# NeurAI-Lab/biHomE

Hardware: AMD Instinct MI355X
Metric: training image-pairs/s (128x128 patch, bs=64 per GPU, full step: fwd+bwd+Adam) (higher is better)
Workload: dtype f32

## Files before the change

bihome_amd/_lib.py:

```python
import ctypes
import os
from ctypes import POINTER, Structure, c_char_p, c_float, c_int, c_int64, c_void_p

_HERE = os.path.dirname(os.path.abspath(__file__))
TUNING = os.environ.get("BIHOME_TUNING") == "1"
_VARIANT = os.environ.get("BIHOME_LIB_VARIANT", "")
LIB_PATH = os.path.join(_HERE, "libbihome_hip_tuning.so" if TUNING else
                        ("libbihome_hip_%s.so" % _VARIANT if _VARIANT.isalnum() else "libbihome_hip.so"))


class BhConvDesc(Structure):
    _fields_ = [(n, c_int) for n in ("N", "Hi", "Wi", "Ci", "Ho", "Wo", "Co", "kh", "kw", "stride", "pad",
                                     "transposed", "in_nchw", "out_nchw", "precision", "w_layout", "route")] + \
               [("a_bound", c_void_p), ("b_bound", c_void_p)]


GEOMETRY_FIELDS = tuple(n for n, _ in BhConvDesc._fields_[:17])
AMAX_FLOATS = 512


class BhPack3x3Job(Structure):
    _fields_ = [("w", c_void_p), ("pf", c_void_p), ("pd", c_void_p), ("Co", c_int), ("Ci", c_int), ("split", c_int),
                ("reserved", c_int)]

# ... 44 lines not shown
    "bh_l2norm_bwd": [P, P, P, c_int, c_int, P, P],
    "bh_relu_bwd": [P, P, c_int64, P, P],
    "bh_oneline_anchor_bwd": [P] * 8 + [c_int, c_int, c_int, c_int, P, c_int, P, P, P],
    "bh_bihome_anchor_bwd": [P] * 10 + [c_int, c_int, c_int, c_float, c_int, P, P, P],
    "bh_warp_bwd_img": [P, P, c_int, c_int, c_int, c_int, P, P, c_int, P],
    "bh_photo_warp_fwd": [P, P, P, c_int, c_int, c_int, c_int, c_int, P, c_int, P],
    "bh_photo_warp_bwd": [P, P, P, P, c_int, c_int, c_int, c_int, c_int, P, c_int, P],
    "bh_mask_fwd": [P, P, c_int, c_int, c_float, P, P, P, P, P],
    "bh_mask_bwd": [P] * 7 + [c_int, c_int, c_float, P, P, P],
    "bh_conv3x3_pack": [P, c_int, P],
    "bh_conv3x3_pack_f16": [P, c_int, P],
    "bh_absmax": [P, c_int64, P, P],
    "bh_bn_fwd_coeffs": [P, P, P, P, P, c_int, c_int, c_int, c_float, c_float, P, P, P],
    "bh_bn_fwd": [P] * 8 + [c_int, c_int, c_int, c_float, c_float, c_int, c_int, P, P],
    "bh_bn_bwd": [P] * 11 + [c_int, c_int, c_int, c_float, c_int, c_int, P, P, P, P],
    "bh_conv_variant": [POINTER(BhConvDesc), c_int, c_int, c_int, c_char_p, c_int],
    "bh_conv_fwd": [P, P, P, P, POINTER(BhConvDesc), P],
    "bh_conv_fwd_act": [P, P, P, P, P, POINTER(BhConvDesc), c_int, P],
    "bh_conv_fwd_amax": [P, P, P, P, POINTER(BhConvDesc), P, P],
    "bh_conv_fwd_bnstats": [P, P, P, P, POINTER(BhConvDesc), P, c_int, P],
    "bh_conv_fwd_bnin": [P, P, P, P, POINTER(BhConvDesc), P, c_int, POINTER(BhBnIn), P],
    "bh_conv_wgrad_bnin": [P, P, P, P, POINTER(BhConvDesc), P, c_int64, POINTER(BhBnIn), P],
    "bh_conv_dgrad": [P, P, P, POINTER(BhConvDesc), c_int, P],
    "bh_conv_dgrad_colsum": [P, P, P, POINTER(BhConvDesc), P, P],
    "bh_bias_grad_from_sums": [P, P, c_int, c_int, P],
    "bh_conv_dgrad_s2": [P, P, P, POINTER(BhConvDesc), c_int, P, P],
    "bh_conv_dgrad_bnreduce": [P, P, P, POINTER(BhConvDesc), c_int, POINTER(BhBnReduce), P, c_int, P],
    "bh_col2im_c1": [P, P, POINTER(BhConvDesc), c_int, P],
    "bh_stem7_dgrad_c1": [P, P, P, POINTER(BhConvDesc), P],
    "bh_stem7_dgrad_c1_warp": [P, P, P, POINTER(BhConvDesc), P, P, P, c_int, P, P],
# ... 74 lines not shown
```

bihome_amd/csrc/bn.hip:

```cpp
#include "common.h"

#define BN_MAX_CHUNKS 256

struct BnGeom {
    int groups, rows, C, C4, LPR, RPP, nchunks, rows_per_chunk;
    int det;
};

static bool bn_geom(int groups, int rows, int C, BnGeom& g, int det) {
    if (C % 4 || groups < 1 || rows < 1) return false;
    g.groups = groups; g.rows = rows; g.C = C; g.C4 = C / 4; g.det = det;
    if (g.C4 > 256 || (256 % g.C4)) return false;
    g.LPR = g.C4; g.RPP = 256 / g.LPR;
    int n = rows / (g.RPP * 4);
    if (n < 1) n = 1;
    if (n > BN_MAX_CHUNKS) n = BN_MAX_CHUNKS;
    g.rows_per_chunk = (rows + n - 1) / n;
    g.nchunks = (rows + g.rows_per_chunk - 1) / g.rows_per_chunk;
    return true;
}

template <int NV>
__device__ __forceinline__ void reduce_rows(double (&v)[NV], int LPR, int RPP, double* sm ) {
    for (int i = 0; i < NV; ++i) sm[threadIdx.x * NV + i] = v[i];
// ... 82 lines not shown
}
__device__ __forceinline__ void bn_coeffs_from_raw(const BnRaw& r, int use_running, float eps, double inv_rows, float& mean,
                                                   float& invstd, float& scale, float& shift) {
    if (use_running) { mean = (float)r.s1; invstd = 1.0f / sqrtf((float)r.s2 + eps); }
    else {
        const double m = r.s1 * inv_rows;
        double var = r.s2 * inv_rows - m * m;
        if (var < 0) var = 0;
        mean = (float)m;
        invstd = 1.0f / sqrtf((float)var + eps);
    }
    scale = r.gm * invstd;
    shift = r.bt - mean * scale;
}

__global__ void __launch_bounds__(256) bn_apply_kernel(const float* __restrict__ x, const float* __restrict__ gamma,
                                                       const float* __restrict__ beta, const float* __restrict__ rmean,
                                                       const float* __restrict__ rvar, const float* __restrict__ res,
                                                       float* __restrict__ y, const double* __restrict__ stats, BnGeom g,
                                                       float eps, int flags, int use_running, float momentum,
                                                       float* __restrict__ upd_mean, float* __restrict__ upd_var,
                                                       unsigned* __restrict__ amax) {
    __shared__ float sm_amax[4];
    float vmax = 0.f;
    const int cq = threadIdx.x % g.LPR, r0 = threadIdx.x / g.LPR;
    const int grp = blockIdx.y;
    BnRaw raw[4];
#pragma unroll
    for (int i = 0; i < 4; ++i) raw[i] = bn_raw(stats, gamma, beta, rmean, rvar, use_running, g.groups, grp, g.C, cq * 4 + i, g.det);
    const size_t gbase = ((size_t)grp * g.rows) * g.C + cq * 4;
    const bool relu = flags & 1, addres = (flags & 2) && res;
    const int stride = gridDim.x * g.RPP;
    int r = blockIdx.x * g.RPP + r0;
    float4 a[4], q[4];
#pragma unroll
    for (int u = 0; u < 4; ++u) {
        const int rr = r + u * stride;
// ... 3 lines not shown
    float sc[4], sh[4];
    const double inv_rows = 1.0 / (double)g.rows;
#pragma unroll
    for (int i = 0; i < 4; ++i) {
        float m, is;
        bn_coeffs_from_raw(raw[i], use_running, eps, inv_rows, m, is, sc[i], sh[i]);
    }
    if (upd_mean && blockIdx.x == 0 && blockIdx.y == 0) bn_update_running(stats, g, momentum, upd_mean, upd_var);
    while (true) {
#pragma unroll
        for (int u = 0; u < 4; ++u) {
            const int rr = r + u * stride;
            if (rr >= g.rows) break;
            float4 o = make_float4(a[u].x * sc[0] + sh[0], a[u].y * sc[1] + sh[1], a[u].z * sc[2] + sh[2], a[u].w * sc[3] + sh[3]);
            if (addres) { o.x += q[u].x; o.y += q[u].y; o.z += q[u].z; o.w += q[u].w; }
            if (relu) { o.x = fmaxf(o.x, 0.f); o.y = fmaxf(o.y, 0.f); o.z = fmaxf(o.z, 0.f); o.w = fmaxf(o.w, 0.f); }
            *reinterpret_cast<float4*>(y + gbase + (size_t)rr * g.C) = o;
            vmax = fmaxf(fmaxf(vmax, fmaxf(fabsf(o.x), fabsf(o.y))), fmaxf(fabsf(o.z), fabsf(o.w)));
        }
        r += 4 * stride;
        if (r >= g.rows) break;
#pragma unroll
        for (int u = 0; u < 4; ++u) {
            const int rr = r + u * stride;
            a[u] = rr < g.rows ? *reinterpret_cast<const float4*>(x + gbase + (size_t)rr * g.C) : make_float4(0.f, 0.f, 0.f, 0.f);
            q[u] = (addres && rr < g.rows) ? *reinterpret_cast<const float4*>(res + gbase + (size_t)rr * g.C) : make_float4(0.f, 0.f, 0.f, 0.f);
        }
    }
    if (amax) bh_amax_commit(amax, vmax, blockIdx.x + blockIdx.y * 7u, sm_amax);
}

__global__ void __launch_bounds__(256) bn_bwd_reduce_kernel(const float* __restrict__ gy, const float* __restrict__ y,
                                                            const float* __restrict__ x, const float* __restrict__ gamma,
                                                            const float* __restrict__ beta, const double* __restrict__ stats,
                                                            const float* __restrict__ rmean, const float* __restrict__ rvar,
                                                            BnGeom g, float eps, int flags, int use_running,
                                                            double* __restrict__ part) {
    __shared__ double sm[256 * 8];
    const int cq = threadIdx.x % g.LPR, r0 = threadIdx.x / g.LPR;
    const int grp = blockIdx.y, chunk = blockIdx.x;
    const int rbeg = chunk * g.rows_per_chunk, rend = min(g.rows, rbeg + g.rows_per_chunk);
    float mean[4], invstd[4], sc[4], sh[4];
#pragma unroll
    for (int i = 0; i < 4; ++i)
        bn_coeffs(stats, gamma, beta, rmean, rvar, use_running, g.groups, grp, g.C, cq * 4 + i, eps, (double)g.rows, mean[i], invstd[i], sc[i], sh[i], g.det);
    const size_t gbase = ((size_t)grp * g.rows) * g.C + cq * 4;
    const bool relu = flags & 1, mask_from_x = flags & 4;
    double v[8] = {0, 0, 0, 0, 0, 0, 0, 0};
    const bool need_y = relu && !mask_from_x;
    auto accumulate = [&](float4 d, const float4& a, const float4& yv) {
        if (relu) {
            float4 o;
            if (mask_from_x) o = make_float4(a.x * sc[0] + sh[0], a.y * sc[1] + sh[1], a.z * sc[2] + sh[2], a.w * sc[3] + sh[3]);
            else o = yv;
            if (!(o.x > 0.f)) d.x = 0.f;
            if (!(o.y > 0.f)) d.y = 0.f;
            if (!(o.z > 0.f)) d.z = 0.f;
            if (!(o.w > 0.f)) d.w = 0.f;
        }
        v[0] += d.x; v[1] += d.y; v[2] += d.z; v[3] += d.w;
        v[4] += (double)(d.x * ((a.x - mean[0]) * invstd[0]));
        v[5] += (double)(d.y * ((a.y - mean[1]) * invstd[1]));
        v[6] += (double)(d.z * ((a.z - mean[2]) * invstd[2]));
        v[7] += (double)(d.w * ((a.w - mean[3]) * invstd[3]));
    };
    int r = rbeg + r0;
    for (; r + 3 * g.RPP < rend; r += 4 * g.RPP) {
        float4 d[4], a[4], yv[4];
#pragma unroll
        for (int u = 0; u < 4; ++u) {
            const size_t off = gbase + (size_t)(r + u * g.RPP) * g.C;
            d[u] = *reinterpret_cast<const float4*>(gy + off);
            a[u] = *reinterpret_cast<const float4*>(x + off);
            yv[u] = need_y ? *reinterpret_cast<const float4*>(y + off) : make_float4(0.f, 0.f, 0.f, 0.f);
        }
#pragma unroll
        for (int u = 0; u < 4; ++u) accumulate(d[u], a[u], yv[u]);
    }
    for (; r < rend; r += g.RPP) {
        const size_t off = gbase + (size_t)r * g.C;
        const float4 d = *reinterpret_cast<const float4*>(gy + off);
        const float4 a = *reinterpret_cast<const float4*>(x + off);
        const float4 yv = need_y ? *reinterpret_cast<const float4*>(y + off) : make_float4(0.f, 0.f, 0.f, 0.f);
        accumulate(d, a, yv);
    }
    reduce_rows<8>(v, g.LPR, g.RPP, sm);
    if ((int)threadIdx.x < g.LPR) {
        double* p = part + (((size_t)grp * g.nchunks + chunk) * g.C + cq * 4) * 2;
        for (int i = 0; i < 4; ++i) { p[i * 2] = v[i]; p[i * 2 + 1] = v[4 + i]; }
    }
}

__global__ void __launch_bounds__(64) bn_bwd_finalize_kernel(const double* __restrict__ part, BnGeom g,
                                                             const double* __restrict__ stats, const float* __restrict__ rmean,
                                                             const float* __restrict__ rvar, float eps, int use_running,
                                                             float* __restrict__ ggamma, float* __restrict__ gbeta,
                                                             float4* __restrict__ coef) {
    const int c = blockIdx.x, lane = threadIdx.x;
    double tg = 0, tb = 0;
// ... 7 lines not shown
        if (lane == 0) {
            float mean, invstd, sc, sh;
            bn_coeffs(stats, nullptr, nullptr, rmean, rvar, use_running, g.groups, grp, g.C, c, eps, (double)g.rows, mean, invstd, sc, sh, g.det);
            const float invn = 1.0f / (float)g.rows;
            coef[(size_t)grp * g.C + c] = use_running ? make_float4(mean, invstd, 0.f, 0.f)
                                                      : make_float4(mean, invstd, (float)s1 * invn, (float)s2 * invn);
        }
        tb += s1; tg += s2;
    }
    if (lane == 0) {
        if (ggamma) ggamma[c] += (float)tg;
        if (gbeta) gbeta[c] += (float)tb;
    }
}

__global__ void __launch_bounds__(256) bn_bwd_apply_kernel(const float* __restrict__ gy, const float* __restrict__ y,
                                                           const float* __restrict__ x, const float* __restrict__ gamma,
                                                           const float* __restrict__ beta,
                                                           const float4* __restrict__ coef,
                                                           float* __restrict__ gx, float* __restrict__ gres, BnGeom g,
                                                           int flags, const double* __restrict__ stats,
                                                           const double* __restrict__ sums, float eps,
                                                           float* __restrict__ ggamma, float* __restrict__ gbeta,
                                                           unsigned* __restrict__ amax) {
    __shared__ float sm_amax[4];
    float vmax = 0.f;
    const int cq = threadIdx.x % g.LPR, r0 = threadIdx.x / g.LPR;
    const int grp = blockIdx.y;
    BnRaw raw[4];
    float4 cf4[4];
    double rs1[4], rs2[4];
#pragma unroll
    for (int i = 0; i < 4; ++i) {
        const int c = cq * 4 + i;
        cf4[i] = make_float4(0.f, 0.f, 0.f, 0.f); rs1[i] = 0; rs2[i] = 0;
        if (coef) {
            cf4[i] = coef[(size_t)grp * g.C + c];
            raw[i].gm = gamma ? gamma[c] : 1.f; raw[i].bt = beta ? beta[c] : 0.f; raw[i].s1 = 0; raw[i].s2 = 0;
        } else {
            raw[i] = bn_raw(stats, gamma, beta, nullptr, nullptr, 0, g.groups, grp, g.C, c, g.det);
            rs1[i] = bn_sum_total(sums, g.groups, grp, g.C, c, 0, g.det);
            rs2[i] = bn_sum_total(sums, g.groups, grp, g.C, c, 1, g.det);
        }
    }
    const size_t gbase = ((size_t)grp * g.rows) * g.C + cq * 4;
    const bool relu = flags & 1, mask_from_x = flags & 4;
    const bool rd_y = relu && !mask_from_x;
    const int stride = gridDim.x * g.RPP;
    int r = blockIdx.x * g.RPP + r0;
    float4 dv[4], av[4], yv[4];
    auto issue = [&](int rb) {
#pragma unroll
        for (int u = 0; u < 4; ++u) {
            const int rr = rb + u * stride;
            const size_t off = gbase + (size_t)rr * g.C;
            const bool ok = rr < g.rows;
            dv[u] = ok ? *reinterpret_cast<const float4*>(gy + off) : make_float4(0.f, 0.f, 0.f, 0.f);
            av[u] = ok ? *reinterpret_cast<const float4*>(x + off) : make_float4(0.f, 0.f, 0.f, 0.f);
            yv[u] = (ok && rd_y) ? *reinterpret_cast<const float4*>(y + off) : make_float4(0.f, 0.f, 0.f, 0.f);
        }
    };
    issue(r);
    float mean[4], invstd[4], sc[4], sh[4], k1[4], k2[4];
    const double inv_rows = 1.0 / (double)g.rows;
    const float invn = 1.0f / (float)g.rows;
#pragma unroll
    for (int i = 0; i < 4; ++i) {
        if (coef) {
            mean[i] = cf4[i].x; invstd[i] = cf4[i].y; k1[i] = cf4[i].z; k2[i] = cf4[i].w;
            sc[i] = raw[i].gm * cf4[i].y;
            sh[i] = raw[i].bt - cf4[i].x * sc[i];
        } else {
            bn_coeffs_from_raw(raw[i], 0, eps, inv_rows, mean[i], invstd[i], sc[i], sh[i]);
            k1[i] = (float)rs1[i] * invn;
// ... 11 lines not shown
            if (gbeta) gbeta[c] += (float)tb;
        }
    }
    while (true) {
#pragma unroll
        for (int u = 0; u < 4; ++u) {
            const int rr = r + u * stride;
            if (rr >= g.rows) break;
            const size_t off = gbase + (size_t)rr * g.C;
            float4 d = dv[u];
            const float4 a = av[u];
            if (relu) {
                float4 o;
                if (mask_from_x) o = make_float4(a.x * sc[0] + sh[0], a.y * sc[1] + sh[1], a.z * sc[2] + sh[2], a.w * sc[3] + sh[3]);
                else o = yv[u];
                if (!(o.x > 0.f)) d.x = 0.f;
                if (!(o.y > 0.f)) d.y = 0.f;
                if (!(o.z > 0.f)) d.z = 0.f;
                if (!(o.w > 0.f)) d.w = 0.f;
            }
            if (gres) *reinterpret_cast<float4*>(gres + off) = d;
            float4 o;
            o.x = sc[0] * (d.x - k1[0] - (a.x - mean[0]) * invstd[0] * k2[0]);
            o.y = sc[1] * (d.y - k1[1] - (a.y - mean[1]) * invstd[1] * k2[1]);
            o.z = sc[2] * (d.z - k1[2] - (a.z - mean[2]) * invstd[2] * k2[2]);
            o.w = sc[3] * (d.w - k1[3] - (a.w - mean[3]) * invstd[3] * k2[3]);
            *reinterpret_cast<float4*>(gx + off) = o;
            vmax = fmaxf(fmaxf(vmax, fmaxf(fabsf(o.x), fabsf(o.y))), fmaxf(fabsf(o.z), fabsf(o.w)));
        }
        r += 4 * stride;
        if (r >= g.rows) break;
        issue(r);
    }
    if (amax) bh_amax_commit(amax, vmax, blockIdx.x + blockIdx.y * 7u, sm_amax);
// ... 338 lines not shown
}

int bn1_fwd(const float* x, const float* gamma, const float* beta, float* running_mean, float* running_var, const float* res, float* y,
            double* stats, int groups, int rows, float eps, float momentum, int flags, int use_running, hipStream_t s);
int bn1_bwd(const float* gy, const float* y, const float* x, const float* gamma, const float* beta, const double* stats, float* gx,
            float* gres, float* ggamma, float* gbeta, double* scratch, int groups, int rows, float eps, int flags, int use_running,
            const float* running_mean, const float* running_var, hipStream_t s);

extern "C" {

int bh_bn_stats_doubles(int groups, int C) { return (int)BH_BN_SUM_DOUBLES(groups, C); }

int bh_bn_fwd(const float* x, const float* gamma, const float* beta, float* running_mean, float* running_var,
              const float* res, float* y, double* stats, int groups, int rows, int C, float eps, float momentum,
              int flags, int use_running, float* amax_y, void* stream) {
    BnGeom g;
    if (!x || !y || !stats) return BH_E_BADARG;
    if (use_running && (!running_mean || !running_var)) return BH_E_BADARG;
    if (C == 1) return amax_y ? BH_E_UNSUPPORTED : bn1_fwd(x, gamma, beta, running_mean, running_var, res, y, stats, groups, rows, eps, momentum, flags, use_running, bh_stream(stream));
    if (!bn_geom(groups, rows, C, g, (flags & BH_BN_DETERMINISTIC) ? 1 : 0)) return BH_E_UNSUPPORTED;
    hipStream_t s = bh_stream(stream);
    if (!use_running && !(flags & 8)) {
        hipLaunchKernelGGL(bn_stats_kernel, dim3(g.nchunks, groups), dim3(256), 0, s, x, g, stats);
        BH_LAUNCH_CHECK();
    }
    const bool upd = !use_running && running_mean && running_var;
    hipLaunchKernelGGL(bn_apply_kernel, dim3(apply_blocks(g), groups), dim3(256), 0, s, x, gamma, beta, running_mean,
                       running_var, res, y, stats, g, eps, flags, use_running, momentum, upd ? running_mean : nullptr,
                       upd ? running_var : nullptr, reinterpret_cast<unsigned*>(amax_y));
    BH_LAUNCH_CHECK();
    return BH_OK;
}

int bh_bn_fwd_coeffs(const double* stats, const float* gamma, const float* beta, float* running_mean, float* running_var, int groups,
                     int rows, int C, float eps, float momentum, float* table, float* amax_y, void* stream) {
    BnGeom g;
    if (!stats || !table) return BH_E_BADARG;
    if (!bn_geom(groups, rows, C, g, -1)) return BH_E_UNSUPPORTED;
    const bool upd = running_mean && running_var;
    hipLaunchKernelGGL(bn_fwd_coeffs_kernel, dim3((groups * C + 255) / 256 + (upd ? 1 : 0)), dim3(256), 0, bh_stream(stream), stats, gamma, beta, g, eps,
                       momentum, upd ? running_mean : nullptr, upd ? running_var : nullptr, reinterpret_cast<float2*>(table),
                       reinterpret_cast<unsigned*>(amax_y));
    BH_LAUNCH_CHECK();
    return BH_OK;
}

int bh_bn_bwd(const float* gy, const float* y, const float* x, const float* gamma, const float* beta, const double* stats, float* gx,
              float* gres, float* ggamma, float* gbeta, double* scratch, int groups, int rows, int C, float eps, int flags,
              int use_running, const float* running_mean, const float* running_var, float* amax_gx, void* stream) {
    BnGeom g;
    if (!gy || !x || !gx || !stats || !scratch || ((flags & 1) && !(flags & 4) && !y)) return BH_E_BADARG;
    if ((flags & 4) && (flags & 2)) return BH_E_BADARG;
    if (C == 1) return amax_gx ? BH_E_UNSUPPORTED : bn1_bwd(gy, y, x, gamma, beta, stats, gx, gres, ggamma, gbeta, scratch, groups, rows, eps, flags, use_running,
                               running_mean, running_var, bh_stream(stream));
    if (!bn_geom(groups, rows, C, g, (flags & BH_BN_DETERMINISTIC) ? 1 : 0)) return BH_E_UNSUPPORTED;
    hipStream_t s = bh_stream(stream);
    if (flags & 16) {
        if (use_running) return BH_E_BADARG;
        hipLaunchKernelGGL(bn_bwd_apply_kernel, dim3(apply_blocks(g), groups), dim3(256), 0, s, gy, y, x, gamma, beta,
                           (const float4*)nullptr, gx, gres, g, flags, stats, (const double*)scratch, eps, ggamma, gbeta,
                           reinterpret_cast<unsigned*>(amax_gx));
        BH_LAUNCH_CHECK();
        return BH_OK;
    }
    float4* coef = reinterpret_cast<float4*>(scratch);
    double* part = scratch + (size_t)groups * C * 2;
    const bool need_sums = !use_running || ggamma || gbeta;
    if (need_sums) {
        hipLaunchKernelGGL(bn_bwd_reduce_kernel, dim3(g.nchunks, groups), dim3(256), 0, s, gy, y, x, gamma, beta, stats,
                           running_mean, running_var, g, eps, flags, use_running, part);
        BH_LAUNCH_CHECK();
    }
    BnGeom gf = g;
    if (!need_sums) gf.nchunks = 0;
    hipLaunchKernelGGL(bn_bwd_finalize_kernel, dim3(C), dim3(64), 0, s, part, gf, stats, running_mean, running_var, eps,
                       use_running, ggamma, gbeta, coef);
    BH_LAUNCH_CHECK();
    hipLaunchKernelGGL(bn_bwd_apply_kernel, dim3(apply_blocks(g), groups), dim3(256), 0, s, gy, y, x, gamma, beta, coef,
                       gx, gres, g, flags, (const double*)nullptr, (const double*)nullptr, eps, (float*)nullptr,
                       (float*)nullptr, reinterpret_cast<unsigned*>(amax_gx));
    BH_LAUNCH_CHECK();
    return BH_OK;
}

int bh_bn_scratch_doubles(int groups, int C) { return groups * C * 2 * (1 + (BN_MAX_CHUNKS > 256 ? BN_MAX_CHUNKS : 256)); }

int bh_bn_stats(const float* x, double* stats, int groups, int rows, int C, int flags, void* stream) {
    if (!x || !stats) return BH_E_BADARG;
    return bn_launch_stats(x, groups, rows, C, stats, bh_stream(stream), (flags & BH_BN_DETERMINISTIC) ? 1 : 0);
}

int bh_bn_maxpool_fwd(const float* x, const float* gamma, const float* beta, float* running_mean, float* running_var, float* y,
                      unsigned char* idx, double* stats, int groups, int N, int Hi, int Wi, int C, float eps, float momentum, int flags,
                      int use_running, float* amax_y, void* stream) {
    BnGeom g;
// ... 409 lines not shown
```

bihome_amd/kernels.py:

```python
import ctypes
import os

import torch

from ._lib import (AMAX_FLOATS, BN_DETERMINISTIC, DSAC_METHODS, F_DETERMINISTIC, GEOMETRY_FIELDS, ROUTE_DETERMINISTIC, ROUTE_WX3_PC, ROUTE_WX3_SHARED, BhBnIn, BhBnReduce, BhConvDesc,
                   BhPack3x3Job, check, lib)


def _p(t):
    return None if t is None else ctypes.c_void_p(t.data_ptr())


_DET_DEFAULT = os.environ.get("BIHOME_DETERMINISTIC", "0") == "1"
_DET_SCOPE = []


def set_deterministic(on=True):
    global _DET_DEFAULT
    prev, _DET_DEFAULT = _DET_DEFAULT, bool(on)
    return prev


def deterministic():
    return _DET_SCOPE[-1] if _DET_SCOPE else _DET_DEFAULT
# ... 984 lines not shown
            check(lib.bh_conv_bias_grad(_p(gy), _p(gbias), ctypes.byref(d), _stream()), "bh_conv_bias_grad")


BN_SUM_STRIDE = 16
BN_SUM_SLOTS = 1


def bn_stats_doubles(groups, C):
    return BN_SUM_SLOTS * groups * C * 2 * BN_SUM_STRIDE


def bn_stats_buffer(groups, C, device):
    return torch.zeros(lib.bh_bn_stats_doubles(groups, C), dtype=torch.float64, device=device)


def bn_fwd(x, gamma, beta, rmean, rvar, res, groups, eps, momentum, relu, training, stats=None, stats_ready=False, amax=None):
    _chk(x); _chk(res)
    C = gamma.numel() if gamma is not None else x.shape[-1]
    rows = x.numel() // C // groups
    y = torch.empty_like(x)
    if stats is None:
        stats = bn_stats_buffer(groups, C, x.device)
        stats_ready = False
    flags = (1 if relu else 0) | (2 if res is not None else 0) | (8 if stats_ready else 0) | (BN_DETERMINISTIC if deterministic() else 0)
    nb = 4.0 * x.numel() * ((2 if (training and not stats_ready) else 1) + 1 + (1 if res is not None else 0))
    with _Timed("bn_fwd(%d kernels)" % (2 if (training and not stats_ready) else 1) + (" g%d rows%d C%d" % (groups, rows, C) if TIMING_DETAIL else ""), 0.0, nb):
        check(lib.bh_bn_fwd(_p(x), _p(gamma), _p(beta), _p(rmean), _p(rvar), _p(res), _p(y), _p(stats), groups, rows, C,
                            float(eps), float(momentum), flags, 0 if training else 1, _p(amax), _stream()), "bh_bn_fwd")
    if amax is not None:
        y._bh_amax = amax
    return y, stats


def bn_bwd(gy, y, x, gamma, stats, rmean, rvar, groups, eps, relu, training, want_gres, ggamma=None, gbeta=None, beta=None,
           had_res=None, scratch=None, sums_ready=None, amax=None):
    _chk(gy); _chk(x)
    C = gamma.numel() if gamma is not None else x.shape[-1]
    rows = x.numel() // C // groups
    gx = torch.empty_like(x)
    gres = torch.empty_like(x) if want_gres else None
    if sums_ready is not None:
        scratch = sums_ready
    elif scratch is None:
        scratch = torch.empty(lib.bh_bn_scratch_doubles(groups, C), dtype=torch.float64, device=x.device)
    had_res = want_gres if had_res is None else had_res
    mask_from_x = relu and not had_res
    flags = ((1 if relu else 0) | (2 if want_gres else 0) | (4 if mask_from_x else 0) | (16 if sums_ready is not None else 0)
             | (BN_DETERMINISTIC if deterministic() else 0))
    passes = 1 if sums_ready is not None else 2
    nb = 4.0 * x.numel() * (passes * (2 + (1 if (relu and not mask_from_x) else 0)) + 1 + (1 if want_gres else 0))
    with _Timed("bn_bwd(%d kernels)" % (1 if sums_ready is not None else 3) + (" g%d rows%d C%d" % (groups, rows, C) if TIMING_DETAIL else ""), 0.0, nb):
        check(lib.bh_bn_bwd(_p(gy), _p(y), _p(x), _p(gamma), _p(beta), _p(stats), _p(gx), _p(gres), _p(ggamma), _p(gbeta),
                            _p(scratch), groups, rows, C, float(eps), flags, 0 if training else 1, _p(rmean), _p(rvar),
                            _p(amax), _stream()), "bh_bn_bwd")
    if amax is not None:
        gx._bh_amax = amax
    return gx, gres


def bn_stats(x, stats, groups, C):
    _chk(x); _chk(stats, torch.float64)
    rows = x.numel() // C // groups
    with _Timed("bn_stats_kernel", 0.0, 4.0 * x.numel()):
        check(lib.bh_bn_stats(_p(x), _p(stats), groups, rows, C, BN_DETERMINISTIC if deterministic() else 0, _stream()), "bh_bn_stats")
    return stats


class BnPooled:
    __slots__ = ("pooled", "idx", "shape")
# ... 200 lines not shown
```

bihome_amd/net.py:

```python
import os
import weakref

import torch
import torch.nn as nn

from . import kernels as K
from . import plan as P


def to_kernel_layout_(module):
    for m in module.modules():
        if isinstance(m, (nn.Conv2d, nn.ConvTranspose2d)):
            if not m.weight.data.is_contiguous(memory_format=torch.channels_last):
                m.weight.data = m.weight.data.contiguous(memory_format=torch.channels_last)
    return module


def kview(w):
    if w.dim() == 2:
        return w
    v = w.permute(0, 2, 3, 1)
    if not v.is_contiguous():
        raise RuntimeError("conv weight is not in kernel (channels_last) layout; call net.to_kernel_layout_(module)")
    return v
# ... 151 lines not shown
            low = self.sequential(src, blk.lower_branch)
        up = list(blk.upper_branch)
        assert isinstance(up[-1], nn.BatchNorm2d)
        mid = self.sequential(src, up[:-1])
        return self.bn(mid, up[-1], relu=True, res=low)

    def basic_block(self, src, blk):
        low = src
        if blk.downsample is not None:
            low = self.sequential(src, blk.downsample)
        t = self.bn(self.conv(src, blk.conv1), blk.bn1, relu=True)
        return self.bn(self.conv(t, blk.conv2), blk.bn2, relu=True, res=low)


class Ctx:
    __slots__ = ("slots", "stats", "descs", "groups", "training", "weights", "wkeys", "wpacked", "precision", "joined")

    def __init__(self):
        self.slots, self.stats, self.descs, self.weights, self.wkeys, self.wpacked = {}, {}, {}, {}, {}, {}
        self.joined = {}
        self.precision = 0


_GEOM_CACHE = {}
X3_WS_BYTES = 40 << 20
DET_WS_BYTES = 256 << 20


def _conv_geometry(mod, x_shape, in_nchw, out_nchw, precision=0):
    key = (id(mod), tuple(x_shape), bool(in_nchw), bool(out_nchw), int(precision), K.deterministic())
    hit = _GEOM_CACHE.get(key)
    if hit is not None and hit[0] is mod:
        return hit[1]
    d = _conv_geometry_uncached(mod, x_shape, in_nchw, out_nchw, precision)
    d.bh_packs = bool(isinstance(mod, nn.Conv2d) and K.packs_3x3(d))
# ... 153 lines not shown
    else:
        if isinstance(res, K.BnJoinPending):
            lo, _ = K.bn_fwd(res.x, res.mod.weight, res.mod.bias, res.mod.running_mean, res.mod.running_var, None, groups, res.mod.eps,
                             _momentum(res.mod), False, training, stats=res.stats, stats_ready=True)
            res = s.slots[op.res] = lo
        st = _bn_stats_slice(s, i, m.num_features)
        if i in plan.bn_pool and src.dim() == 4 and src.shape[0] % groups == 0:
            out = K.bn_maxpool_fwd(src, m.weight, m.bias, m.running_mean, m.running_var, groups, m.eps, _momentum(m), op.relu,
                                   training, st, i in s.ready, want_index=s.save, amax=amax_next() if amax_next else None)
        elif _bn_on_load_ok(s, i, op, src):
            rec = amax_next() if amax_next else None
            table = K.bn_fwd_coeffs(st, m.weight, m.bias, m.running_mean, m.running_var, groups,
                                    src.numel() // (m.num_features * groups), m.num_features, m.eps, _momentum(m), amax=rec)
            out = K.BnOnLoad(src, table, groups, op.relu, amax=rec)
        else:
            out, st = K.bn_fwd(src, m.weight, m.bias, m.running_mean, m.running_var, res, groups, m.eps, _momentum(m), op.relu, training,
                               stats=st, stats_ready=i in s.ready, amax=amax_next() if (amax_next and m.num_features > 1) else None)
    if training:
        _count_batch(m, groups)
    if s.save:
        s.ctx.stats[i] = st
    return out


def _fw_tail(s, i, op, src):
    c1, bn, c2 = op.mod
    N, h, w, _ = src.shape
    out, ws = K.tail_fwd(src, kview(c1.weight), c1.bias, bn.weight, bn.bias, bn.running_mean, bn.running_var,
                         kview(c2.weight), c2.bias, s.groups, h * w, bn.eps, _momentum(bn), s.training)
    if s.training:
        _count_batch(bn, s.groups)
    if s.save:
# ... 163 lines not shown
    train_w = s.want_wgrad and m.weight is not None and m.weight.requires_grad
    ggamma, gbeta = (m.weight.grad, m.bias.grad) if train_w else (None, None)
    amax = amax_next() if (amax_next and m.num_features > 1) else None
    gres = None
    if isinstance(g, K.GradFrom1x1):
        gx = K.bn_bwd_from_1x1(g, x, m.weight, m.bias, ctx.stats[i], ctx.groups, m.eps, op.relu, ggamma, gbeta, amax=amax)
    elif isinstance(g, K.PooledGrad):
        gx = K.bn_maxpool_bwd(g, x, m.weight, m.bias, ctx.stats[i], m.running_mean, m.running_var, ctx.groups, m.eps, op.relu,
                              ctx.training, ggamma, gbeta, amax=amax)
    else:
        yb = s.slots[op.dst]
        if isinstance(yb, (K.BnOnLoad, K.BnPooled)):
            yb = None
        gx, gres = K.bn_bwd(g, yb, x, m.weight, ctx.stats[i], m.running_mean, m.running_var, ctx.groups,
                            m.eps, op.relu, ctx.training, op.res is not None and ((op.res != 0) or s.want_input_grad),
                            ggamma, gbeta, beta=m.bias, had_res=op.res is not None, sums_ready=s.bn_reduced.get(i), amax=amax)
    if train_w and s.on_param_grad is not None:
        s.on_param_grad(m.weight)
        s.on_param_grad(m.bias)
    if need_src_grad:
        _contribute(s.grads, op.src, gx)
    if gres is not None:
        _contribute(s.grads, op.res, gres)


def _bw_tail(s, i, op, g, x, need_src_grad):
    ctx = s.ctx
    c1, bn, c2 = op.mod
    tr = s.want_wgrad and c1.weight.requires_grad
    N, h, w, _ = x.shape
    eval_b1 = tr and not ctx.training and c1.bias is not None and c1.bias.requires_grad
# ... 216 lines not shown
```

bihome_amd/plan.py:

```python
import torch.nn as nn

from . import kernels as K


class ProgramIndex:
    __slots__ = ("nops", "producer", "consumers", "users", "consumer", "last_consumer")

    def __init__(self, ops):
        self.nops = len(ops)
        self.producer = {op.dst: j for j, op in enumerate(ops)}
        self.consumers = {}
        self.consumer = {}
        for j, op in enumerate(ops):
            self.consumers.setdefault(op.src, []).append(j)
            if op.res is not None:
                self.consumers.setdefault(op.res, []).append(j)
            self.consumer.setdefault(op.src, j)
        self.users = {s: len(v) for s, v in self.consumers.items()}
        self.last_consumer = {s: v[0] for s, v in self.consumers.items()}


def packs_weight(op, device=None):
    m = op.mod
    return (op.kind == "conv" and isinstance(m, nn.Conv2d) and op.extra["weight_fn"] is None and m.kernel_size == (3, 3)
            and m.stride == (1, 1) and m.padding == (1, 1) and m.in_channels % 32 == 0 and m.out_channels % 32 == 0
            and (device is None or m.weight.device == device))


def packed_weight_ids(prog):
    return {id(op.mod.weight) for op in prog.ops if packs_weight(op)}


class ForwardPlan:
    __slots__ = ("nops", "fused_stats", "bn_on_load", "bn_on_load_1x1", "joins", "join_lower", "consumer", "bn_pool", "folded", "deferred",
                 "bn_off", "total", "nrec")


def forward_key(prog, training, groups, precision, packer, fold):
    return (bool(training), int(groups), int(precision), packer.serial if packer is not None else 0,
            len(packer.entries) if packer is not None else 0, bool(packer.f16) if packer is not None else False,
            tuple(op.mod.weight.requires_grad for op in prog.ops if op.kind == "conv"), bool(fold))


def plan_fused_stats(prog, ix, training):
    fused_stats = {}
    if training:
        ops = prog.ops
        for i, op in enumerate(ops):
            j = ix.producer.get(op.src)
            if (op.kind == "bn" and j is not None and ops[j].kind == "conv" and ix.users.get(op.src, 0) == 1
# ... 34 lines not shown
    return out


def plan_joins(prog, ix, training, bn_on_load):
    joins = {}
    if training:
        ops = prog.ops
        for i, op in enumerate(ops):
            j = ix.producer.get(op.res) if (op.kind == "bn" and op.res is not None) else None
            if (j is not None and ops[j].kind == "bn" and ops[j].res is None and not ops[j].relu
                    and ix.users.get(op.res, 0) == 1 and j not in bn_on_load and i not in bn_on_load
                    and op.mod.num_features == ops[j].mod.num_features and op.mod.num_features % 4 == 0
                    and op.mod.weight is not None and ops[j].mod.weight is not None):
                joins[i] = j
    return joins


def plan_bn_pool(prog, ix):
    ops = prog.ops
    return {i for i, op in enumerate(ops[:-1])
            if op.kind == "bn" and op.res is None and ops[i + 1].kind == "maxpool" and ops[i + 1].src == op.dst
            and op.mod.num_features % 4 == 0 and op.mod.num_features > 1 and ix.users.get(op.dst, 0) == 1}


def plan_folded(prog, ix, fold):
    folded = {}
    if fold:
        ops = prog.ops
        for i, op in enumerate(ops):
            j = ix.producer.get(op.src)
# ... 13 lines not shown
    if int(precision) == K.F16X2:
        nrec = max(1, sum(1 for op in prog.ops if op.kind == "bn" or (op.kind == "conv" and isinstance(op.mod, nn.ConvTranspose2d))))
    return bn_off, total, nrec


def make_forward_plan(prog, training, groups, precision, packed_ids=None, fold=False):
    ix = prog.index()
    p = ForwardPlan()
    p.nops = ix.nops
    p.fused_stats = plan_fused_stats(prog, ix, training)
    p.bn_on_load_1x1 = plan_bn_on_load_1x1(prog, ix, training, groups, precision, p.fused_stats)
    p.bn_on_load = plan_bn_on_load(prog, ix, training, groups, precision, packed_ids, p.fused_stats)
    p.consumer = ix.consumer if (training and packed_ids is not None and int(precision) in K.SPLIT_PIECES) else None
    p.joins = plan_joins(prog, ix, training, p.bn_on_load)
    p.join_lower = set(p.joins.values())
    p.bn_pool = plan_bn_pool(prog, ix)
    p.folded = plan_folded(prog, ix, fold)
    p.deferred = set(p.folded.values())
    p.bn_off, p.total, p.nrec = plan_forward_arenas(prog, groups, precision)
    return p


def forward_plan(prog, training, groups, precision, packer, fold):
    key = forward_key(prog, training, groups, precision, packer, fold)
    p = prog.fw_plans.get(key)
    if p is None:
        if len(prog.fw_plans) > 16:
            prog.fw_plans.clear()
        p = prog.fw_plans[key] = make_forward_plan(prog, training, groups, precision,
                                                   set(packer.entries) if packer is not None else None, fold)
# ... 93 lines not shown
```

include/bihome.h:

```cpp
#ifndef BIHOME_H
#define BIHOME_H

#include <stdint.h>

#ifdef __cplusplus
extern "C" {
#endif

#define BH_OK 0
#define BH_E_BADARG (-1)
#define BH_E_UNSUPPORTED (-2)

int bh_version(void);
int bh_device_arch(char* buf, int buflen);

#define BH_F_DETERMINISTIC 1
#define BH_BN_DETERMINISTIC 32
int bh_probe_mfma_bf16(int random_operands, float* sink_dev, double* tflops, void* stream);
int bh_probe_mfma_f32(int random_operands, float* sink_dev, double* tflops, void* stream);


int bh_h4pt_fwd(const float* delta, int B, float W, float H, double* H64, float* H32, void* stream);
int bh_h4pt_bwd(const float* delta, const double* H64, const double* gH, int B, float W, float H,
                float* gdelta, void* stream);
// ... 174 lines not shown
int bh_conv_wgrad(const float* x, const float* gy, float* gw, float* gbias, const bh_conv_desc* d, void* stream);
long long bh_conv_wgrad_det_bytes(const bh_conv_desc* d);
int bh_conv_wgrad_det(const float* x, const float* gy, float* gw, float* gbias, const bh_conv_desc* d, float* ws, long long ws_bytes,
                      void* stream);
int bh_conv_bias_grad(const float* gy, float* gbias, const bh_conv_desc* d, void* stream);

int bh_bn_stats_doubles(int groups, int C);
int bh_bn_scratch_doubles(int groups, int C);
int bh_bn_fwd(const float* x, const float* gamma, const float* beta, float* running_mean, float* running_var,
              const float* res, float* y, double* stats, int groups, int rows, int C, float eps, float momentum,
              int flags, int use_running, float* amax_y, void* stream);
int bh_bn_bwd(const float* gy, const float* y, const float* x, const float* gamma, const float* beta, const double* stats,
              float* gx, float* gres, float* ggamma, float* gbeta, double* scratch,
              int groups, int rows, int C, float eps, int flags, int use_running,
              const float* running_mean, const float* running_var, float* amax_gx, void* stream);

int bh_bn_maxpool_fwd(const float* x, const float* gamma, const float* beta, float* running_mean, float* running_var, float* y,
                      unsigned char* idx, double* stats, int groups, int N, int Hi, int Wi, int C, float eps, float momentum, int flags,
                      int use_running, float* amax_y, void* stream);
int bh_bn_maxpool_bwd(const float* gy, const unsigned char* idx, const float* x, const float* gamma, const float* beta, const double* stats,
                      float* gx, float* ggamma, float* gbeta, double* scratch, int groups, int N, int Hi, int Wi, int C, float eps, int flags,
                      int use_running, const float* running_mean, const float* running_var, float* amax_gx, void* stream);
int bh_bn_bwd_from_1x1(const float* gs, const float* w, int KC, const float* x, const float* gamma, const float* beta, const double* stats,
                       float* gx, float* ggamma, float* gbeta, double* scratch, int groups, int rows, int C, float eps, int flags,
                       float* amax_gx, void* stream);
int bh_bn_stats(const float* x, double* stats, int groups, int rows, int C, int flags, void* stream);
int bh_bn_join_scratch_doubles(int groups, int C);
int bh_bn_join_fwd(const float* xa, const float* xb, const float* gamma_a, const float* beta_a, float* rmean_a, float* rvar_a,
                   const float* gamma_b, const float* beta_b, float* rmean_b, float* rvar_b, const double* stats_a, const double* stats_b,
                   float* y, int groups, int rows, int C, float eps_a, float eps_b, float momentum_a, float momentum_b, int flags,
// ... 46 lines not shown
```

Measured before the change: 5328.

## Save packed ReLU sign bits in BN forward, read them in backward

For training BN layers with a residual add and ReLU, the forward apply kernel now also writes one byte per four channels holding the positive-sign mask. The backward reduce and apply kernels read this byte instead of the full float output y to build the ReLU mask. The goal is to cut backward memory traffic, since reading y costs a full extra float stream per pass. The price is a small extra write in forward, an extra buffer kept alive per layer, and byte-sized loads that may coalesce poorly.

```diff
diff --git a/bihome_amd/_lib.py b/bihome_amd/_lib.py
--- a/bihome_amd/_lib.py
+++ b/bihome_amd/_lib.py
@@ -82,6 +82,8 @@
     "bh_bn_fwd_coeffs": [P, P, P, P, P, c_int, c_int, c_int, c_float, c_float, P, P, P],
     "bh_bn_fwd": [P] * 8 + [c_int, c_int, c_int, c_float, c_float, c_int, c_int, P, P],
     "bh_bn_bwd": [P] * 11 + [c_int, c_int, c_int, c_float, c_int, c_int, P, P, P, P],
+    "bh_bn_fwd_signs": [P] * 8 + [c_int, c_int, c_int, c_float, c_float, c_int, c_int, P, P, P],
+    "bh_bn_bwd_signs": [P] * 11 + [c_int, c_int, c_int, c_float, c_int, c_int, P, P, P, P, P],
     "bh_conv_variant": [POINTER(BhConvDesc), c_int, c_int, c_int, c_char_p, c_int],
     "bh_conv_fwd": [P, P, P, P, POINTER(BhConvDesc), P],
     "bh_conv_fwd_act": [P, P, P, P, P, POINTER(BhConvDesc), c_int, P],
diff --git a/bihome_amd/csrc/bn.hip b/bihome_amd/csrc/bn.hip
--- a/bihome_amd/csrc/bn.hip
+++ b/bihome_amd/csrc/bn.hip
@@ -120,13 +120,18 @@
     shift = r.bt - mean * scale;
 }
 
+__device__ __forceinline__ unsigned char bn_sign_byte(const float4& o) {
+    return (unsigned char)((o.x > 0.f ? 1 : 0) | (o.y > 0.f ? 2 : 0) | (o.z > 0.f ? 4 : 0) | (o.w > 0.f ? 8 : 0));
+}
+
+template <bool SIGNS>
 __global__ void __launch_bounds__(256) bn_apply_kernel(const float* __restrict__ x, const float* __restrict__ gamma,
                                                        const float* __restrict__ beta, const float* __restrict__ rmean,
                                                        const float* __restrict__ rvar, const float* __restrict__ res,
                                                        float* __restrict__ y, const double* __restrict__ stats, BnGeom g,
                                                        float eps, int flags, int use_running, float momentum,
                                                        float* __restrict__ upd_mean, float* __restrict__ upd_var,
-                                                       unsigned* __restrict__ amax) {
+                                                       unsigned* __restrict__ amax, unsigned char* __restrict__ signs) {
     __shared__ float sm_amax[4];
     float vmax = 0.f;
     const int cq = threadIdx.x % g.LPR, r0 = threadIdx.x / g.LPR;
@@ -160,6 +165,7 @@
             if (rr >= g.rows) break;
             float4 o = make_float4(a[u].x * sc[0] + sh[0], a[u].y * sc[1] + sh[1], a[u].z * sc[2] + sh[2], a[u].w * sc[3] + sh[3]);
             if (addres) { o.x += q[u].x; o.y += q[u].y; o.z += q[u].z; o.w += q[u].w; }
+            if (SIGNS) signs[(gbase + (size_t)rr * g.C) >> 2] = bn_sign_byte(o);
             if (relu) { o.x = fmaxf(o.x, 0.f); o.y = fmaxf(o.y, 0.f); o.z = fmaxf(o.z, 0.f); o.w = fmaxf(o.w, 0.f); }
             *reinterpret_cast<float4*>(y + gbase + (size_t)rr * g.C) = o;
             vmax = fmaxf(fmaxf(vmax, fmaxf(fabsf(o.x), fabsf(o.y))), fmaxf(fabsf(o.z), fabsf(o.w)));
@@ -176,12 +182,13 @@
     if (amax) bh_amax_commit(amax, vmax, blockIdx.x + blockIdx.y * 7u, sm_amax);
 }
 
+template <bool SIGNS>
 __global__ void __launch_bounds__(256) bn_bwd_reduce_kernel(const float* __restrict__ gy, const float* __restrict__ y,
                                                             const float* __restrict__ x, const float* __restrict__ gamma,
                                                             const float* __restrict__ beta, const double* __restrict__ stats,
                                                             const float* __restrict__ rmean, const float* __restrict__ rvar,
                                                             BnGeom g, float eps, int flags, int use_running,
-                                                            double* __restrict__ part) {
+                                                            double* __restrict__ part, const unsigned char* __restrict__ signs) {
     __shared__ double sm[256 * 8];
     const int cq = threadIdx.x % g.LPR, r0 = threadIdx.x / g.LPR;
     const int grp = blockIdx.y, chunk = blockIdx.x;
@@ -193,16 +200,17 @@
     const size_t gbase = ((size_t)grp * g.rows) * g.C + cq * 4;
     const bool relu = flags & 1, mask_from_x = flags & 4;
     double v[8] = {0, 0, 0, 0, 0, 0, 0, 0};
-    const bool need_y = relu && !mask_from_x;
-    auto accumulate = [&](float4 d, const float4& a, const float4& yv) {
+    const bool rd_s = SIGNS && relu && !mask_from_x;
+    const bool need_y = relu && !mask_from_x && !rd_s;
+    auto accumulate = [&](float4 d, const float4& a, const float4& yv, unsigned sb) {
         if (relu) {
             float4 o;
             if (mask_from_x) o = make_float4(a.x * sc[0] + sh[0], a.y * sc[1] + sh[1], a.z * sc[2] + sh[2], a.w * sc[3] + sh[3]);
             else o = yv;
-            if (!(o.x > 0.f)) d.x = 0.f;
-            if (!(o.y > 0.f)) d.y = 0.f;
-            if (!(o.z > 0.f)) d.z = 0.f;
-            if (!(o.w > 0.f)) d.w = 0.f;
+            if (!(rd_s ? (sb & 1u) != 0 : o.x > 0.f)) d.x = 0.f;
+            if (!(rd_s ? (sb & 2u) != 0 : o.y > 0.f)) d.y = 0.f;
+            if (!(rd_s ? (sb & 4u) != 0 : o.z > 0.f)) d.z = 0.f;
+            if (!(rd_s ? (sb & 8u) != 0 : o.w > 0.f)) d.w = 0.f;
         }
         v[0] += d.x; v[1] += d.y; v[2] += d.z; v[3] += d.w;
         v[4] += (double)(d.x * ((a.x - mean[0]) * invstd[0]));
@@ -213,22 +221,24 @@
     int r = rbeg + r0;
     for (; r + 3 * g.RPP < rend; r += 4 * g.RPP) {
         float4 d[4], a[4], yv[4];
+        unsigned sv[4];
 #pragma unroll
         for (int u = 0; u < 4; ++u) {
             const size_t off = gbase + (size_t)(r + u * g.RPP) * g.C;
             d[u] = *reinterpret_cast<const float4*>(gy + off);
             a[u] = *reinterpret_cast<const float4*>(x + off);
             yv[u] = need_y ? *reinterpret_cast<const float4*>(y + off) : make_float4(0.f, 0.f, 0.f, 0.f);
-        }
-#pragma unroll
-        for (int u = 0; u < 4; ++u) accumulate(d[u], a[u], yv[u]);
+            sv[u] = rd_s ? signs[off >> 2] : 0u;
+        }
+#pragma unroll
+        for (int u = 0; u < 4; ++u) accumulate(d[u], a[u], yv[u], sv[u]);
     }
     for (; r < rend; r += g.RPP) {
         const size_t off = gbase + (size_t)r * g.C;
         const float4 d = *reinterpret_cast<const float4*>(gy + off);
         const float4 a = *reinterpret_cast<const float4*>(x + off);
         const float4 yv = need_y ? *reinterpret_cast<const float4*>(y + off) : make_float4(0.f, 0.f, 0.f, 0.f);
-        accumulate(d, a, yv);
+        accumulate(d, a, yv, rd_s ? signs[off >> 2] : 0u);
     }
     reduce_rows<8>(v, g.LPR, g.RPP, sm);
     if ((int)threadIdx.x < g.LPR) {
@@ -266,6 +276,7 @@
     }
 }
 
+template <bool SIGNS>
 __global__ void __launch_bounds__(256) bn_bwd_apply_kernel(const float* __restrict__ gy, const float* __restrict__ y,
                                                            const float* __restrict__ x, const float* __restrict__ gamma,
                                                            const float* __restrict__ beta,
@@ -274,7 +285,7 @@
                                                            int flags, const double* __restrict__ stats,
                                                            const double* __restrict__ sums, float eps,
                                                            float* __restrict__ ggamma, float* __restrict__ gbeta,
-                                                           unsigned* __restrict__ amax) {
+                                                           unsigned* __restrict__ amax, const unsigned char* __restrict__ signs) {
     __shared__ float sm_amax[4];
     float vmax = 0.f;
     const int cq = threadIdx.x % g.LPR, r0 = threadIdx.x / g.LPR;
@@ -297,10 +308,12 @@
     }
     const size_t gbase = ((size_t)grp * g.rows) * g.C + cq * 4;
     const bool relu = flags & 1, mask_from_x = flags & 4;
-    const bool rd_y = relu && !mask_from_x;
+    const bool rd_s = SIGNS && relu && !mask_from_x;
+    const bool rd_y = relu && !mask_from_x && !rd_s;
     const int stride = gridDim.x * g.RPP;
     int r = blockIdx.x * g.RPP + r0;
     float4 dv[4], av[4], yv[4];
+    unsigned sv[4];
     auto issue = [&](int rb) {
 #pragma unroll
         for (int u = 0; u < 4; ++u) {
@@ -310,6 +323,7 @@
             dv[u] = ok ? *reinterpret_cast<const float4*>(gy + off) : make_float4(0.f, 0.f, 0.f, 0.f);
             av[u] = ok ? *reinterpret_cast<const float4*>(x + off) : make_float4(0.f, 0.f, 0.f, 0.f);
             yv[u] = (ok && rd_y) ? *reinterpret_cast<const float4*>(y + off) : make_float4(0.f, 0.f, 0.f, 0.f);
+            sv[u] = (ok && rd_s) ? signs[off >> 2] : 0u;
         }
     };
     issue(r);
@@ -351,10 +365,11 @@
                 float4 o;
                 if (mask_from_x) o = make_float4(a.x * sc[0] + sh[0], a.y * sc[1] + sh[1], a.z * sc[2] + sh[2], a.w * sc[3] + sh[3]);
                 else o = yv[u];
-                if (!(o.x > 0.f)) d.x = 0.f;
-                if (!(o.y > 0.f)) d.y = 0.f;
-                if (!(o.z > 0.f)) d.z = 0.f;
-                if (!(o.w > 0.f)) d.w = 0.f;
+                const unsigned sb = sv[u];
+                if (!(rd_s ? (sb & 1u) != 0 : o.x > 0.f)) d.x = 0.f;
+                if (!(rd_s ? (sb & 2u) != 0 : o.y > 0.f)) d.y = 0.f;
+                if (!(rd_s ? (sb & 4u) != 0 : o.z > 0.f)) d.z = 0.f;
+                if (!(rd_s ? (sb & 8u) != 0 : o.w > 0.f)) d.w = 0.f;
             }
             if (gres) *reinterpret_cast<float4*>(gres + off) = d;
             float4 o;
@@ -723,10 +738,17 @@
 int bh_bn_fwd(const float* x, const float* gamma, const float* beta, float* running_mean, float* running_var,
               const float* res, float* y, double* stats, int groups, int rows, int C, float eps, float momentum,
               int flags, int use_running, float* amax_y, void* stream) {
+    return bh_bn_fwd_signs(x, gamma, beta, running_mean, running_var, res, y, stats, groups, rows, C, eps, momentum, flags, use_running,
+                           amax_y, nullptr, stream);
+}
+
+int bh_bn_fwd_signs(const float* x, const float* gamma, const float* beta, float* running_mean, float* running_var,
+                    const float* res, float* y, double* stats, int groups, int rows, int C, float eps, float momentum,
+                    int flags, int use_running, float* amax_y, unsigned char* signs, void* stream) {
     BnGeom g;
     if (!x || !y || !stats) return BH_E_BADARG;
     if (use_running && (!running_mean || !running_var)) return BH_E_BADARG;
-    if (C == 1) return amax_y ? BH_E_UNSUPPORTED : bn1_fwd(x, gamma, beta, running_mean, running_var, res, y, stats, groups, rows, eps, momentum, flags, use_running, bh_stream(stream));
+    if (C == 1) return (amax_y || signs) ? BH_E_UNSUPPORTED : bn1_fwd(x, gamma, beta, running_mean, running_var, res, y, stats, groups, rows, eps, momentum, flags, use_running, bh_stream(stream));
     if (!bn_geom(groups, rows, C, g, (flags & BH_BN_DETERMINISTIC) ? 1 : 0)) return BH_E_UNSUPPORTED;
     hipStream_t s = bh_stream(stream);
     if (!use_running && !(flags & 8)) {
@@ -734,9 +756,9 @@
         BH_LAUNCH_CHECK();
     }
     const bool upd = !use_running && running_mean && running_var;
-    hipLaunchKernelGGL(bn_apply_kernel, dim3(apply_blocks(g), groups), dim3(256), 0, s, x, gamma, beta, running_mean,
+    hipLaunchKernelGGL(signs ? bn_apply_kernel<true> : bn_apply_kernel<false>, dim3(apply_blocks(g), groups), dim3(256), 0, s, x, gamma, beta, running_mean,
                        running_var, res, y, stats, g, eps, flags, use_running, momentum, upd ? running_mean : nullptr,
-                       upd ? running_var : nullptr, reinterpret_cast<unsigned*>(amax_y));
+                       upd ? running_var : nullptr, reinterpret_cast<unsigned*>(amax_y), signs);
     BH_LAUNCH_CHECK();
     return BH_OK;
 }
@@ -757,18 +779,26 @@
 int bh_bn_bwd(const float* gy, const float* y, const float* x, const float* gamma, const float* beta, const double* stats, float* gx,
               float* gres, float* ggamma, float* gbeta, double* scratch, int groups, int rows, int C, float eps, int flags,
               int use_running, const float* running_mean, const float* running_var, float* amax_gx, void* stream) {
+    return bh_bn_bwd_signs(gy, y, x, gamma, beta, stats, gx, gres, ggamma, gbeta, scratch, groups, rows, C, eps, flags, use_running,
+                           running_mean, running_var, amax_gx, nullptr, stream);
+}
+
+int bh_bn_bwd_signs(const float* gy, const float* y, const float* x, const float* gamma, const float* beta, const double* stats, float* gx,
+                    float* gres, float* ggamma, float* gbeta, double* scratch, int groups, int rows, int C, float eps, int flags,
+                    int use_running, const float* running_mean, const float* running_var, float* amax_gx, const unsigned char* signs,
+                    void* stream) {
     BnGeom g;
-    if (!gy || !x || !gx || !stats || !scratch || ((flags & 1) && !(flags & 4) && !y)) return BH_E_BADARG;
+    if (!gy || !x || !gx || !stats || !scratch || ((flags & 1) && !(flags & 4) && !y && !signs)) return BH_E_BADARG;
     if ((flags & 4) && (flags & 2)) return BH_E_BADARG;
-    if (C == 1) return amax_gx ? BH_E_UNSUPPORTED : bn1_bwd(gy, y, x, gamma, beta, stats, gx, gres, ggamma, gbeta, scratch, groups, rows, eps, flags, use_running,
+    if (C == 1) return (amax_gx || signs) ? BH_E_UNSUPPORTED : bn1_bwd(gy, y, x, gamma, beta, stats, gx, gres, ggamma, gbeta, scratch, groups, rows, eps, flags, use_running,
                                running_mean, running_var, bh_stream(stream));
     if (!bn_geom(groups, rows, C, g, (flags & BH_BN_DETERMINISTIC) ? 1 : 0)) return BH_E_UNSUPPORTED;
     hipStream_t s = bh_stream(stream);
     if (flags & 16) {
         if (use_running) return BH_E_BADARG;
-        hipLaunchKernelGGL(bn_bwd_apply_kernel, dim3(apply_blocks(g), groups), dim3(256), 0, s, gy, y, x, gamma, beta,
+        hipLaunchKernelGGL(signs ? bn_bwd_apply_kernel<true> : bn_bwd_apply_kernel<false>, dim3(apply_blocks(g), groups), dim3(256), 0, s, gy, y, x, gamma, beta,
                            (const float4*)nullptr, gx, gres, g, flags, stats, (const double*)scratch, eps, ggamma, gbeta,
-                           reinterpret_cast<unsigned*>(amax_gx));
+                           reinterpret_cast<unsigned*>(amax_gx), signs);
         BH_LAUNCH_CHECK();
         return BH_OK;
     }
@@ -776,8 +806,8 @@
     double* part = scratch + (size_t)groups * C * 2;
     const bool need_sums = !use_running || ggamma || gbeta;
     if (need_sums) {
-        hipLaunchKernelGGL(bn_bwd_reduce_kernel, dim3(g.nchunks, groups), dim3(256), 0, s, gy, y, x, gamma, beta, stats,
-                           running_mean, running_var, g, eps, flags, use_running, part);
+        hipLaunchKernelGGL(signs ? bn_bwd_reduce_kernel<true> : bn_bwd_reduce_kernel<false>, dim3(g.nchunks, groups), dim3(256), 0, s, gy, y, x, gamma, beta, stats,
+                           running_mean, running_var, g, eps, flags, use_running, part, signs);
         BH_LAUNCH_CHECK();
     }
     BnGeom gf = g;
@@ -785,9 +815,9 @@
     hipLaunchKernelGGL(bn_bwd_finalize_kernel, dim3(C), dim3(64), 0, s, part, gf, stats, running_mean, running_var, eps,
                        use_running, ggamma, gbeta, coef);
     BH_LAUNCH_CHECK();
-    hipLaunchKernelGGL(bn_bwd_apply_kernel, dim3(apply_blocks(g), groups), dim3(256), 0, s, gy, y, x, gamma, beta, coef,
+    hipLaunchKernelGGL(signs ? bn_bwd_apply_kernel<true> : bn_bwd_apply_kernel<false>, dim3(apply_blocks(g), groups), dim3(256), 0, s, gy, y, x, gamma, beta, coef,
                        gx, gres, g, flags, (const double*)nullptr, (const double*)nullptr, eps, (float*)nullptr,
-                       (float*)nullptr, reinterpret_cast<unsigned*>(amax_gx));
+                       (float*)nullptr, reinterpret_cast<unsigned*>(amax_gx), signs);
     BH_LAUNCH_CHECK();
     return BH_OK;
 }
diff --git a/bihome_amd/kernels.py b/bihome_amd/kernels.py
--- a/bihome_amd/kernels.py
+++ b/bihome_amd/kernels.py
@@ -1022,8 +1022,12 @@
     return torch.zeros(lib.bh_bn_stats_doubles(groups, C), dtype=torch.float64, device=device)
 
 
-def bn_fwd(x, gamma, beta, rmean, rvar, res, groups, eps, momentum, relu, training, stats=None, stats_ready=False, amax=None):
-    _chk(x); _chk(res)
+def bn_sign_bytes(x):
+    return torch.empty(x.numel() // 4, dtype=torch.uint8, device=x.device)
+
+
+def bn_fwd(x, gamma, beta, rmean, rvar, res, groups, eps, momentum, relu, training, stats=None, stats_ready=False, amax=None, signs=None):
+    _chk(x); _chk(res); _chk(signs, torch.uint8)
     C = gamma.numel() if gamma is not None else x.shape[-1]
     rows = x.numel() // C // groups
     y = torch.empty_like(x)
@@ -1031,18 +1035,20 @@
         stats = bn_stats_buffer(groups, C, x.device)
         stats_ready = False
     flags = (1 if relu else 0) | (2 if res is not None else 0) | (8 if stats_ready else 0) | (BN_DETERMINISTIC if deterministic() else 0)
-    nb = 4.0 * x.numel() * ((2 if (training and not stats_ready) else 1) + 1 + (1 if res is not None else 0))
+    if signs is not None and signs.numel() != x.numel() // 4:
+        raise ValueError("signs: %d bytes for %d elements" % (signs.numel(), x.numel()))
+    nb = 4.0 * x.numel() * ((2 if (training and not stats_ready) else 1) + 1 + (1 if res is not None else 0) + (1 / 16 if signs is not None else 0))
     with _Timed("bn_fwd(%d kernels)" % (2 if (training and not stats_ready) else 1) + (" g%d rows%d C%d" % (groups, rows, C) if TIMING_DETAIL else ""), 0.0, nb):
-        check(lib.bh_bn_fwd(_p(x), _p(gamma), _p(beta), _p(rmean), _p(rvar), _p(res), _p(y), _p(stats), groups, rows, C,
-                            float(eps), float(momentum), flags, 0 if training else 1, _p(amax), _stream()), "bh_bn_fwd")
+        check(lib.bh_bn_fwd_signs(_p(x), _p(gamma), _p(beta), _p(rmean), _p(rvar), _p(res), _p(y), _p(stats), groups, rows, C,
+                                  float(eps), float(momentum), flags, 0 if training else 1, _p(amax), _p(signs), _stream()), "bh_bn_fwd")
     if amax is not None:
         y._bh_amax = amax
     return y, stats
 
 
 def bn_bwd(gy, y, x, gamma, stats, rmean, rvar, groups, eps, relu, training, want_gres, ggamma=None, gbeta=None, beta=None,
-           had_res=None, scratch=None, sums_ready=None, amax=None):
-    _chk(gy); _chk(x)
+           had_res=None, scratch=None, sums_ready=None, amax=None, signs=None):
+    _chk(gy); _chk(x); _chk(signs, torch.uint8)
     C = gamma.numel() if gamma is not None else x.shape[-1]
     rows = x.numel() // C // groups
     gx = torch.empty_like(x)
@@ -1056,11 +1062,14 @@
     flags = ((1 if relu else 0) | (2 if want_gres else 0) | (4 if mask_from_x else 0) | (16 if sums_ready is not None else 0)
              | (BN_DETERMINISTIC if deterministic() else 0))
     passes = 1 if sums_ready is not None else 2
-    nb = 4.0 * x.numel() * (passes * (2 + (1 if (relu and not mask_from_x) else 0)) + 1 + (1 if want_gres else 0))
+    if signs is not None and signs.numel() != x.numel() // 4:
+        raise ValueError("signs: %d bytes for %d elements" % (signs.numel(), x.numel()))
+    mask_read = 0 if (not relu or mask_from_x) else (1 / 16 if signs is not None else 1)
+    nb = 4.0 * x.numel() * (passes * (2 + mask_read) + 1 + (1 if want_gres else 0))
     with _Timed("bn_bwd(%d kernels)" % (1 if sums_ready is not None else 3) + (" g%d rows%d C%d" % (groups, rows, C) if TIMING_DETAIL else ""), 0.0, nb):
-        check(lib.bh_bn_bwd(_p(gy), _p(y), _p(x), _p(gamma), _p(beta), _p(stats), _p(gx), _p(gres), _p(ggamma), _p(gbeta),
-                            _p(scratch), groups, rows, C, float(eps), flags, 0 if training else 1, _p(rmean), _p(rvar),
-                            _p(amax), _stream()), "bh_bn_bwd")
+        check(lib.bh_bn_bwd_signs(_p(gy), _p(y), _p(x), _p(gamma), _p(beta), _p(stats), _p(gx), _p(gres), _p(ggamma), _p(gbeta),
+                                  _p(scratch), groups, rows, C, float(eps), flags, 0 if training else 1, _p(rmean), _p(rvar),
+                                  _p(amax), _p(signs), _stream()), "bh_bn_bwd")
     if amax is not None:
         gx._bh_amax = amax
     return gx, gres
diff --git a/bihome_amd/net.py b/bihome_amd/net.py
--- a/bihome_amd/net.py
+++ b/bihome_amd/net.py
@@ -189,11 +189,12 @@
 
 
 class Ctx:
-    __slots__ = ("slots", "stats", "descs", "groups", "training", "weights", "wkeys", "wpacked", "precision", "joined")
+    __slots__ = ("slots", "stats", "descs", "groups", "training", "weights", "wkeys", "wpacked", "precision", "joined", "signs")
 
     def __init__(self):
         self.slots, self.stats, self.descs, self.weights, self.wkeys, self.wpacked = {}, {}, {}, {}, {}, {}
         self.joined = {}
+        self.signs = {}
         self.precision = 0
 
 
@@ -377,8 +378,12 @@
                                     src.numel() // (m.num_features * groups), m.num_features, m.eps, _momentum(m), amax=rec)
             out = K.BnOnLoad(src, table, groups, op.relu, amax=rec)
         else:
+            signs = K.bn_sign_bytes(src) if (s.save and i in plan.sign_bytes and res is not None) else None
             out, st = K.bn_fwd(src, m.weight, m.bias, m.running_mean, m.running_var, res, groups, m.eps, _momentum(m), op.relu, training,
-                               stats=st, stats_ready=i in s.ready, amax=amax_next() if (amax_next and m.num_features > 1) else None)
+                               stats=st, stats_ready=i in s.ready, amax=amax_next() if (amax_next and m.num_features > 1) else None,
+                               signs=signs)
+            if signs is not None:
+                s.ctx.signs[i] = signs
     if training:
         _count_batch(m, groups)
     if s.save:
@@ -572,7 +577,8 @@
             yb = None
         gx, gres = K.bn_bwd(g, yb, x, m.weight, ctx.stats[i], m.running_mean, m.running_var, ctx.groups,
                             m.eps, op.relu, ctx.training, op.res is not None and ((op.res != 0) or s.want_input_grad),
-                            ggamma, gbeta, beta=m.bias, had_res=op.res is not None, sums_ready=s.bn_reduced.get(i), amax=amax)
+                            ggamma, gbeta, beta=m.bias, had_res=op.res is not None, sums_ready=s.bn_reduced.get(i), amax=amax,
+                            signs=ctx.signs.get(i))
     if train_w and s.on_param_grad is not None:
         s.on_param_grad(m.weight)
         s.on_param_grad(m.bias)
diff --git a/bihome_amd/plan.py b/bihome_amd/plan.py
--- a/bihome_amd/plan.py
+++ b/bihome_amd/plan.py
@@ -32,8 +32,8 @@
 
 
 class ForwardPlan:
-    __slots__ = ("nops", "fused_stats", "bn_on_load", "bn_on_load_1x1", "joins", "join_lower", "consumer", "bn_pool", "folded", "deferred",
-                 "bn_off", "total", "nrec")
+    __slots__ = ("nops", "fused_stats", "bn_on_load", "bn_on_load_1x1", "joins", "join_lower", "sign_bytes", "consumer", "bn_pool", "folded",
+                 "deferred", "bn_off", "total", "nrec")
 
 
 def forward_key(prog, training, groups, precision, packer, fold):
@@ -98,6 +98,16 @@
                     and op.mod.weight is not None and ops[j].mod.weight is not None):
                 joins[i] = j
     return joins
+
+
+def plan_sign_bytes(prog, ix, training, joins, bn_on_load):
+    out = set()
+    if training:
+        for i, op in enumerate(prog.ops):
+            if (op.kind == "bn" and op.res is not None and op.relu and i not in joins and i not in bn_on_load
+                    and op.mod.num_features % 4 == 0):
+                out.add(i)
+    return out
 
 
 def plan_bn_pool(prog, ix):
@@ -141,6 +151,7 @@
     p.consumer = ix.consumer if (training and packed_ids is not None and int(precision) in K.SPLIT_PIECES) else None
     p.joins = plan_joins(prog, ix, training, p.bn_on_load)
     p.join_lower = set(p.joins.values())
+    p.sign_bytes = plan_sign_bytes(prog, ix, training, p.joins, p.bn_on_load)
     p.bn_pool = plan_bn_pool(prog, ix)
     p.folded = plan_folded(prog, ix, fold)
     p.deferred = set(p.folded.values())
diff --git a/include/bihome.h b/include/bihome.h
--- a/include/bihome.h
+++ b/include/bihome.h
@@ -212,6 +212,13 @@
               float* gx, float* gres, float* ggamma, float* gbeta, double* scratch,
               int groups, int rows, int C, float eps, int flags, int use_running,
               const float* running_mean, const float* running_var, float* amax_gx, void* stream);
+int bh_bn_fwd_signs(const float* x, const float* gamma, const float* beta, float* running_mean, float* running_var,
+                    const float* res, float* y, double* stats, int groups, int rows, int C, float eps, float momentum,
+                    int flags, int use_running, float* amax_y, unsigned char* signs, void* stream);
+int bh_bn_bwd_signs(const float* gy, const float* y, const float* x, const float* gamma, const float* beta, const double* stats,
+                    float* gx, float* gres, float* ggamma, float* gbeta, double* scratch,
+                    int groups, int rows, int C, float eps, int flags, int use_running,
+                    const float* running_mean, const float* running_var, float* amax_gx, const unsigned char* signs, void* stream);
 
 int bh_bn_maxpool_fwd(const float* x, const float* gamma, const float* beta, float* running_mean, float* running_var, float* y,
                       unsigned char* idx, double* stats, int groups, int N, int Hi, int Wi, int C, float eps, float momentum, int flags,
```

Measured after the change: 5342, median of 3. Within noise of the previous version (+0.3%).
